# akanazawa/human_dynamics

Hardware: NVIDIA H100
Metric: frames/sec (ResNet->f_movie->SMPL LBS) (higher is better)
Workload: dtype f32 (wgmma 3x fp16 head/remainder split, fp32 two-level accumulate)

## Files before the change

human_dynamics_b200/_lib.py:

```python
from __future__ import annotations

import ctypes as C
import os

_HERE = os.path.dirname(os.path.abspath(__file__))
LIB_PATH = os.path.join(_HERE, 'libhd_b200.so')

HD_IMPL_SIMT, HD_IMPL_TC_3XTF32, HD_IMPL_TC_1XTF32, HD_IMPL_TC_3XF16 = 0, 1, 2, 3
HD_CONV_NO_TMA_EPILOGUE = 1
HD_CONV_INPUT_PLANES = 2
HD_PACK_FORWARD, HD_PACK_BACKWARD_DATA = 0, 1
IMPL_BY_NAME = {'simt': HD_IMPL_SIMT, 'tc3': HD_IMPL_TC_3XTF32, 'tc1': HD_IMPL_TC_1XTF32, 'tc3h': HD_IMPL_TC_3XF16}


class ConvDesc(C.Structure):
    _fields_ = [
        ('in_', C.c_void_p), ('in_ld', C.c_longlong),
        ('n_img', C.c_int), ('H', C.c_int), ('W', C.c_int), ('Cin', C.c_int),
        ('Ho', C.c_int), ('Wo', C.c_int), ('KH', C.c_int), ('KW', C.c_int),
        ('stride', C.c_int), ('pad_t', C.c_int), ('pad_l', C.c_int),
        ('w_kn', C.c_void_p), ('w_nk_hi', C.c_void_p), ('w_nk_lo', C.c_void_p),
        ('Cout', C.c_int), ('K_pad', C.c_int),
        ('pre_scale', C.c_void_p), ('pre_shift', C.c_void_p), ('pre_img_stride', C.c_int), ('pre_relu', C.c_int),
        ('post_scale', C.c_void_p), ('post_shift', C.c_void_p), ('post_relu', C.c_int),
        ('res', C.c_void_p), ('res_ld', C.c_longlong), ('res_H', C.c_int), ('res_W', C.c_int), ('res_stride', C.c_int),
        ('out', C.c_void_p), ('out_ld', C.c_longlong),
        ('impl', C.c_int),
        ('tmap_hi', C.c_void_p), ('tmap_lo', C.c_void_p),
        ('in_hi', C.c_void_p), ('in_lo', C.c_void_p),
        ('out_hi', C.c_void_p), ('out_lo', C.c_void_p), ('out2_ld', C.c_longlong),
        ('post2_scale', C.c_void_p), ('post2_shift', C.c_void_p), ('post2_relu', C.c_int),
        ('tmap_res', C.c_void_p), ('tmap_out', C.c_void_p), ('tmap_out_hi', C.c_void_p), ('tmap_out_lo', C.c_void_p),
        ('flags', C.c_int),
# ... 206 lines not shown
```

human_dynamics_b200/csrc/conv_common.cuh:

```cuda
#pragma once
#include <cuda_fp16.h>
#include "common.cuh"

namespace hd {

struct ConvParams {
  const float *in; long long in_ld;
  int n_img, H, W, Cin, Ho, Wo, KH, KW, stride, pad_t, pad_l;
  const float *w_kn; int Cout; int K; int M;
  const float *pre_scale, *pre_shift; int pre_img_stride, pre_relu;
  const float *post_scale, *post_shift; int post_relu;
  const float *res; long long res_ld; int res_H, res_W, res_stride;
  float *out; long long out_ld;
  int vec_out;
  int K_pad;
  const void *in_hi, *in_lo;
  void *out_hi, *out_lo; long long out2_ld;
  const float *post2_scale, *post2_shift; int post2_relu;
  int out_sub;
  int planes;
  long long *dbg;
};

#ifdef __CUDACC__
// ... 29 lines not shown
    return HD_ERR_INVALID;
  }
  p.in = d->in; p.in_ld = d->in_ld;
  p.n_img = d->n_img; p.H = d->H; p.W = d->W; p.Cin = d->Cin; p.Ho = d->Ho; p.Wo = d->Wo;
  p.KH = d->KH; p.KW = d->KW; p.stride = d->stride; p.pad_t = d->pad_t; p.pad_l = d->pad_l;
  p.w_kn = d->w_kn; p.Cout = d->Cout; p.K = d->KH * d->KW * d->Cin;
  const long long M = (long long)d->n_img * d->Ho * d->Wo;
  if (M > 0x7fffffffLL) { set_last_error_text("hd_conv_gemm: M overflows int32"); return HD_ERR_INVALID; }
  p.M = (int)M;
  p.pre_scale = d->pre_scale; p.pre_shift = d->pre_shift; p.pre_img_stride = d->pre_img_stride; p.pre_relu = d->pre_relu;
  p.post_scale = d->post_scale; p.post_shift = d->post_shift; p.post_relu = d->post_relu;
  p.res = d->res; p.res_ld = d->res_ld; p.res_H = d->res_H; p.res_W = d->res_W; p.res_stride = d->res_stride;
  p.out = d->out; p.out_ld = d->out_ld;
  p.in_hi = d->in_hi; p.in_lo = d->in_lo; p.out_hi = d->out_hi; p.out_lo = d->out_lo; p.out2_ld = d->out2_ld;
  p.post2_scale = d->post2_scale; p.post2_shift = d->post2_shift; p.post2_relu = d->post2_relu;
  p.vec_out = (d->Cout % 4 == 0) && (!d->out || ((d->out_ld % 4 == 0) && aligned16(d->out))) &&
              (!d->out_hi || ((d->out2_ld % 4 == 0) && aligned16(d->out_hi) && aligned16(d->out_lo))) &&
              (!d->res || ((d->res_ld % 4 == 0) && aligned16(d->res))) &&
              (!d->post_scale || aligned16(d->post_scale)) && (!d->post_shift || aligned16(d->post_shift));
  p.K_pad = d->K_pad;
  p.planes = (d->flags & HD_CONV_INPUT_PLANES) ? 1 : 0;
  p.out_sub = d->out_subsample > 1 ? d->out_subsample : 0;
  if (p.out_sub && !d->out) { set_last_error_text("hd_conv_gemm: out_subsample needs `out`"); return HD_ERR_INVALID; }
  p.dbg = nullptr;
  return HD_OK;
}

int launch_conv_simt(const ConvParams &p, cudaStream_t st);
int launch_conv_tc(const ConvParams &p, const hd_conv_desc *d, cudaStream_t st);

}
```

human_dynamics_b200/csrc/conv_tc.cu:

```cuda
#include <cuda.h>
#include <cuda_fp16.h>
#include <cstdlib>
#include "conv_common.cuh"
#include "tc_ptx.cuh"

namespace hd {
namespace {

constexpr int BM = 128;
constexpr int A_TILE_BYTES = BM * 128;
constexpr int BOX_BYTES = 64 * 128;
constexpr int W_PROD = 8;
constexpr int STAGE_OUT = 1, STAGE_PAIR = 2;

using namespace ptx;

template <bool HALF, bool ASPLIT, int BN, bool RES = false>
struct Cfg {
  static_assert(BN == 64 || (BN == 128 && HALF && ASPLIT), "128-wide N tiles: pre-split fp16 path only");
  static_assert(!RES || ASPLIT, "residual by TMA: pre-split fp16 path only");
  static constexpr int PROD_THREADS = BN == 128 ? 128 : 256;
  static constexpr int NUM_THREADS = 256 + PROD_THREADS;
  static constexpr int ROW_STEP = PROD_THREADS / 8;
  static constexpr int ROWS = BM / ROW_STEP;
  static constexpr int PROD_REGS = BN == 128 ? 40 : 104, CONS_REGS = BN == 128 ? 232 : 152;
  static_assert(256 * CONS_REGS + PROD_THREADS * PROD_REGS <= 65536, "setmaxnreg split beyond the register file");
  static constexpr int NACC = BN / 2;
  static constexpr int STAGES = BN == 128 ? (RES ? 2 : 3) : (RES ? 3 : 4);
  static constexpr int BKE = HALF ? 64 : 32;
  static constexpr int B_TILE_BYTES = BN * 128;
  static constexpr int STAGE_BYTES = 2 * A_TILE_BYTES + 2 * B_TILE_BYTES;
  static constexpr int RES_OFFSET = STAGES * STAGE_BYTES;
  static constexpr int RES_SLOT_BYTES = RES ? 64 * BN * 4 : 0;
  static constexpr int STG_OFFSET = RES_OFFSET + 2 * RES_SLOT_BYTES;
  static constexpr int STG_BYTES = ASPLIT ? 2 * BOX_BYTES : 0;
  static constexpr int BAR_OFFSET = STG_OFFSET + 2 * STG_BYTES;
  static constexpr int SMEM_BYTES = BAR_OFFSET + 128 + 1024;
  static_assert(SMEM_BYTES <= 232448, "dynamic shared memory beyond the 227 KB a CTA can opt into");
  static constexpr int PF = HALF ? 2 : 3;
  static constexpr int V = HALF ? 2 : 1;
};

template <int R>
struct RowState {
  int n[R], iy[R], ix[R];
};

template <bool SPLIT, int PCH, bool HALF, bool GATHER, bool ASPLIT, int BN, bool RES>
__global__ void __launch_bounds__((Cfg<HALF, ASPLIT, BN, RES>::NUM_THREADS), 1)
conv_gemm_tc_kernel(const ConvParams p, const __grid_constant__ CUtensorMap tmap_hi, const __grid_constant__ CUtensorMap tmap_lo,
                    const __grid_constant__ CUtensorMap tmap_res, const __grid_constant__ CUtensorMap tmap_out,
                    const __grid_constant__ CUtensorMap tmap_out_hi, const __grid_constant__ CUtensorMap tmap_out_lo, const int stage) {
  using C = Cfg<HALF, ASPLIT, BN, RES>;
  constexpr int BKE = C::BKE, PF = C::PF, V = C::V, STAGES = C::STAGES, R = C::ROWS, RS = C::ROW_STEP, NA = C::NACC;
  extern __shared__ uint8_t smem_raw[];
  const uint32_t smem_base = (smem_u32(smem_raw) + 1023u) & ~1023u;
  uint8_t *smem = smem_raw + (smem_base - smem_u32(smem_raw));
  const uint32_t bar_base = smem_base + C::BAR_OFFSET;
  auto full_bar = [&](int s) { return bar_base + 8u * s; };
  auto empty_bar = [&](int s) { return bar_base + 8u * (STAGES + s); };
  auto res_bar = [&](int g) { return bar_base + 8u * (2 * STAGES + g); };

  const int warp = threadIdx.x >> 5, lane = threadIdx.x & 31;
  const int num_k = (GATHER ? p.K_pad : p.K) / BKE;
  const int tiles_n = (p.Cout + BN - 1) / BN;
  const int num_tiles = ((p.M + BM - 1) / BM) * tiles_n;
  const int my_tiles = (num_tiles - (int)blockIdx.x + (int)gridDim.x - 1) / (int)gridDim.x;

  if (threadIdx.x == 0) {
    for (int s = 0; s < STAGES; ++s) {
      mbar_init(full_bar(s), ASPLIT ? C::PROD_THREADS + 1 : 9);
      mbar_init(empty_bar(s), 8);
    }
    if (RES) for (int g = 0; g < 2; ++g) mbar_init(res_bar(g), 1);
    asm volatile("fence.mbarrier_init.release.cluster;" ::: "memory");
  }
  __syncthreads();
  const int xmode = p.dbg ? (int)p.dbg[15] : 0;

  if (warp >= W_PROD) {
    asm volatile("setmaxnreg.dec.sync.aligned.u32 %0;" ::"n"(C::PROD_REGS));
    const int t = threadIdx.x - W_PROD * 32;
    const int j = t & 7;
    const int rb = t >> 3;
    const uint32_t sw_off = (uint32_t)((j ^ (rb & 7)) << 4);
    const bool prof = p.dbg != nullptr && blockIdx.x == 0 && t == 0;
    long long t_wait = 0, t_start = prof && BN == 64 ? clock64() : 0;
    if (BN == 128 && prof) p.dbg[0] = clock64();
    const int total = my_tiles * num_k;
    auto load_b = [&](int s, int ti, int kc) {
      if (t != 0) return;
      const int n0 = (((int)blockIdx.x + ti * (int)gridDim.x) % tiles_n) * BN;
      const uint32_t b_hi = smem_base + s * C::STAGE_BYTES + 2 * A_TILE_BYTES;
      if (xmode & 2) { mbar_arrive(full_bar(s)); return; }
      const int boxes = (BN == 128 && n0 + 64 < p.Cout) ? 2 : 1;
      mbar_arrive_expect_tx(full_bar(s), (SPLIT ? 2 : 1) * boxes * BOX_BYTES);
      for (int b = 0; b < boxes; ++b) {
// ... 2 lines not shown
      }
    };

    auto enter_tile = [&](int ti, RowState<R> &rs) {
      const int tile = (int)blockIdx.x + ti * (int)gridDim.x;
      const int m0 = (tile / tiles_n) * BM;
      const int hw = p.Ho * p.Wo;
#pragma unroll
      for (int i = 0; i < R; ++i) {
        const int m = m0 + rb + RS * i;
        if (m < p.M) {
          const int n = m / hw;
          const int r = m - n * hw;
          const int oy = r / p.Wo, ox = r - oy * p.Wo;
          rs.n[i] = n; rs.iy[i] = oy * p.stride - p.pad_t; rs.ix[i] = ox * p.stride - p.pad_l;
        } else {
          rs.n[i] = -1; rs.iy[i] = 0; rs.ix[i] = 0;
        }
      }
    };
    if constexpr (ASPLIT) {
      const __half *ihi = reinterpret_cast<const __half *>(p.in_hi);
      const __half *ilo = reinterpret_cast<const __half *>(p.in_lo);
      if (!p.planes && p.KH * p.KW <= 32 && (long long)p.n_img * p.H * p.W * p.in_ld < (1ll << 31)) {
        const uint32_t off0 = (uint32_t)rb * 128u + sw_off;
        int base[R];
        uint32_t mask[R];
        int kc = 0, ti = 0, tap = 0, ci0 = 0, kx = 0, ky = 0, tap_off = 0;
        for (int q = 0; q < total; ++q) {
          if (kc == 0) {
            const int tile = (int)blockIdx.x + ti * (int)gridDim.x;
            const int m0 = (tile / tiles_n) * BM + rb;
            const int hw = p.Ho * p.Wo;
#pragma unroll
            for (int i = 0; i < R; ++i) {
              const int m = m0 + RS * i;
              uint32_t mk = 0;
              int b = 0;
              if (m < p.M) {
                const int n = m / hw;
                const int r = m - n * hw;
                const int oy = r / p.Wo, ox = r - oy * p.Wo;
                const int iy0 = oy * p.stride - p.pad_t, ix0 = ox * p.stride - p.pad_l;
                b = ((n * p.H + iy0) * p.W + ix0) * p.in_ld + j * 8;
                int t = 0;
                for (int yy = 0; yy < p.KH; ++yy)
                  for (int xx = 0; xx < p.KW; ++xx, ++t)
// ... 577 lines not shown
}

constexpr int kMaxDevices = 64;

int encode_epilogue_map(CUtensorMap *tm, bool fp16, const void *base, int cols, int rows, long long ld_bytes, const char *what) {
  EncodeTiledFn fn = get_encode_fn();
  if (!fn) { set_last_error_text("cuTensorMapEncodeTiled unavailable (no CUDA driver?)"); return HD_ERR_UNSUPPORTED; }
  const cuuint64_t gdim[2] = {(cuuint64_t)cols, (cuuint64_t)rows};
  const cuuint64_t gstride[1] = {(cuuint64_t)ld_bytes};
  const cuuint32_t box[2] = {fp16 ? 64u : 32u, 64u};
  const cuuint32_t estr[2] = {1u, 1u};
  CUresult r = fn(tm, fp16 ? CU_TENSOR_MAP_DATA_TYPE_FLOAT16 : CU_TENSOR_MAP_DATA_TYPE_FLOAT32, 2, const_cast<void *>(base), gdim, gstride,
                  box, estr, CU_TENSOR_MAP_INTERLEAVE_NONE, CU_TENSOR_MAP_SWIZZLE_128B, CU_TENSOR_MAP_L2_PROMOTION_L2_128B,
                  CU_TENSOR_MAP_FLOAT_OOB_FILL_NONE);
  if (r != CUDA_SUCCESS) {
    char msg[96];
    snprintf(msg, sizeof(msg), "cuTensorMapEncodeTiled (%s) failed with CUresult %d", what, (int)r);
    set_last_error_text(msg);
    return HD_ERR_CUDA;
  }
  return HD_OK;
}

template <bool SPLIT, int PCH, bool HALF, bool GATHER = false, bool ASPLIT = false, int BN = 64, bool RES = false>
int launch_tc(const ConvParams &p, const hd_conv_desc *d, cudaStream_t st) {
  using C = Cfg<HALF, ASPLIT, BN, RES>;
  static bool configured[kMaxDevices] = {};
  static int num_sms[kMaxDevices] = {};
  int dev = 0;
  cudaGetDevice(&dev);
  if (dev < 0 || dev >= kMaxDevices) { set_last_error_text("conv_gemm_tc: device ordinal out of range"); return HD_ERR_UNSUPPORTED; }
  if (!configured[dev]) {
    cudaError_t e = cudaFuncSetAttribute(conv_gemm_tc_kernel<SPLIT, PCH, HALF, GATHER, ASPLIT, BN, RES>,
                                         cudaFuncAttributeMaxDynamicSharedMemorySize, C::SMEM_BYTES);
    if (e != cudaSuccess) { set_last_error("conv_gemm_tc attr", e); return HD_ERR_CUDA; }
    cudaDeviceGetAttribute(&num_sms[dev], cudaDevAttrMultiProcessorCount, dev);
    if (num_sms[dev] <= 0) { set_last_error_text("conv_gemm_tc: no multiprocessor count"); return HD_ERR_CUDA; }
    configured[dev] = true;
  }
  alignas(64) CUtensorMap thi, tlo;
  const void *mhi = d->tmap_hi_n64 ? d->tmap_hi_n64 : d->tmap_hi;
  const void *mlo = d->tmap_hi_n64 ? d->tmap_lo_n64 : d->tmap_lo;
  memcpy(&thi, mhi, sizeof(CUtensorMap));
  memcpy(&tlo, mlo ? mlo : mhi, sizeof(CUtensorMap));
  alignas(64) CUtensorMap tres, tout, tohi, tolo;
  memcpy(&tres, &thi, sizeof(CUtensorMap));
  memcpy(&tout, &thi, sizeof(CUtensorMap));
  memcpy(&tohi, &thi, sizeof(CUtensorMap));
  memcpy(&tolo, &thi, sizeof(CUtensorMap));
  int rc = HD_OK;
  if (RES) rc = encode_epilogue_map(&tres, false, p.res, p.Cout, p.M, p.res_ld * 4, "residual");
  int stage = 0;
  if (ASPLIT && p.out && !p.out_sub) {
    stage |= STAGE_OUT;
    if (rc == HD_OK) rc = encode_epilogue_map(&tout, false, p.out, p.Cout, p.M, p.out_ld * 4, "output");
  }
  if (ASPLIT && p.out_hi && p.out2_ld % 8 == 0) {
    stage |= STAGE_PAIR;
    if (rc == HD_OK) rc = encode_epilogue_map(&tohi, true, p.out_hi, p.Cout, p.M, p.out2_ld * 2, "output head");
    if (rc == HD_OK) rc = encode_epilogue_map(&tolo, true, p.out_lo, p.Cout, p.M, p.out2_ld * 2, "output remainder");
  }
  if (rc != HD_OK) return rc;
  const int num_tiles = ceil_div(p.M, BM) * ceil_div(p.Cout, BN);
  dim3 grid(num_tiles < num_sms[dev] ? num_tiles : num_sms[dev]);
  conv_gemm_tc_kernel<SPLIT, PCH, HALF, GATHER, ASPLIT, BN, RES>
      <<<grid, C::NUM_THREADS, C::SMEM_BYTES, st>>>(p, thi, tlo, tres, tout, tohi, tolo, stage);
  return check_launch("conv_gemm_tc_kernel");
}

bool wide_n_tile(const ConvParams &p) {
  if (p.Cout <= 64) return false;
  int dev = 0, sms = 0;
  cudaGetDevice(&dev);
  cudaDeviceGetAttribute(&sms, cudaDevAttrMultiProcessorCount, dev);
  if (sms <= 0) return true;
  const long long m_tiles = ceil_div(p.M, BM);
  const long long w128 = (m_tiles * ceil_div(p.Cout, 128) + sms - 1) / sms, w64 = (m_tiles * ceil_div(p.Cout, 64) + sms - 1) / sms;
  return 16 * w128 <= 9 * w64;
}

}

int launch_conv_tc(const ConvParams &p, const hd_conv_desc *d, cudaStream_t st) {
  const bool split_b = d->impl != HD_IMPL_TC_1XTF32;
  if (!d->tmap_hi || (split_b && !d->tmap_lo) || (!d->tmap_hi_n64 && d->tmap_lo_n64) || (d->tmap_hi_n64 && split_b && !d->tmap_lo_n64)) {
    set_last_error_text("hd_conv_gemm(tc): missing tensor maps (tmap_hi/tmap_lo, and tmap_hi_n64/tmap_lo_n64 together or not at all)");
    return HD_ERR_INVALID;
  }
  const bool half = d->impl == HD_IMPL_TC_3XF16;
  const int bke = half ? 64 : 32;
  if (p.out_sub) {
    const bool res_plain = !p.res || (p.res_stride == 1 && p.res_H == p.Ho && p.res_W == p.Wo);
    const bool maps = (!p.res || d->tmap_res) && (!p.out_hi || (d->tmap_out_hi && d->tmap_out_lo));
    if (!p.in_hi || p.planes || !maps || !res_plain || p.Cout % 32 != 0 || (d->flags & HD_CONV_NO_TMA_EPILOGUE)) {
      set_last_error_text("hd_conv_gemm: out_subsample needs the activation-map epilogue (pre-split input, Cout % 32 == 0, activation maps given)");
      return HD_ERR_UNSUPPORTED;
    }
  }
  if ((p.out_hi || p.in_hi) && (!half || !p.vec_out)) {
    set_last_error_text("hd_conv_gemm(tc): pre-split activations need impl 3 and 16-byte aligned, 4-column-multiple outputs");
    return HD_ERR_INVALID;
  }
  if (p.in_hi && p.planes) {
    if (p.Cin != 32 || p.KH != 8 || p.KW != 1 || p.stride != 2 || p.pad_t != 0 || p.pad_l != 0 || p.in_ld != 4 || p.Cout > 64 ||
        p.W % 2 != 0 || 2 * (p.Wo - 1) + 8 > p.W || 2 * (p.Ho - 1) + 7 > p.H || !aligned16(p.in_hi) || !aligned16(p.in_lo) || p.pre_scale) {
      set_last_error_text("hd_conv_gemm(tc planes): needs the conv1 plane geometry (Cin 32, KH 8, KW 1, stride 2, in_ld 4, even W)");
      return HD_ERR_INVALID;
    }
    return launch_tc<true, 2, true, false, true>(p, d, st);
  }
  if (p.in_hi) {
    if (p.Cin % 64 != 0 || p.K % 64 != 0 || p.in_ld % 8 != 0 || !aligned16(p.in_hi) || !aligned16(p.in_lo) || p.pre_scale) {
      set_last_error_text("hd_conv_gemm(tc split-A): needs Cin % 64 == 0, in_ld % 8 == 0, aligned in_hi/in_lo, no prologue");
      return HD_ERR_INVALID;
    }
    const bool res_rows = p.res && p.res_stride == 1 && p.res_H == p.Ho && p.res_W == p.Wo && p.K <= 8 * 64;
    if (wide_n_tile(p))
      return res_rows ? launch_tc<true, 2, true, false, true, 128, true>(p, d, st) : launch_tc<true, 2, true, false, true, 128>(p, d, st);
    return res_rows ? launch_tc<true, 2, true, false, true, 64, true>(p, d, st) : launch_tc<true, 2, true, false, true>(p, d, st);
  }
  if (half && p.Cin % bke != 0) {
    const int segp = (p.KW * p.Cin + 7) & ~7;
    if (p.K_pad % 64 != 0 || p.K_pad < p.KH * segp || p.Cout > 64 || p.pre_scale || p.in_ld != p.Cin) {
      set_last_error_text("hd_conv_gemm(tc gather): needs K_pad % 64 == 0, K_pad >= KH*roundup8(KW*Cin), Cout <= 64, dense pixels, no prologue");
      return HD_ERR_INVALID;
    }
    return launch_tc<true, 2, true, true>(p, d, st);
  }
  if (!p.in || p.Cin % bke != 0 || p.in_ld % 4 != 0 || !aligned16(p.in) || p.K % bke != 0 ||
      (p.pre_scale && (!aligned16(p.pre_scale) || !aligned16(p.pre_shift) || p.pre_img_stride % 4 != 0))) {
    set_last_error_text("hd_conv_gemm(tc): needs Cin % 32 (tf32) / % 64 (fp16) == 0 and 16-byte aligned input / prologue vectors");
    return HD_ERR_INVALID;
// ... 55 lines not shown
```

human_dynamics_b200/csrc/net_plan.cu:

```cuda
#include "common.cuh"

#include <algorithm>
#include <cmath>
#include <cstdint>
#include <deque>
#include <functional>
#include <string>
#include <utility>
#include <vector>

struct hd_net {
  int kind = 0;
  hd_weight_fn get = nullptr;
  void *user = nullptr;
  std::vector<void *> allocs;
  std::deque<std::vector<unsigned char>> wmaps;
  std::deque<std::vector<unsigned char>> maps;
  std::vector<std::function<int(cudaStream_t)>> steps;
  std::string err;
  const float *in0 = nullptr;
  float *out0 = nullptr, *out1 = nullptr;
  int n = 0, size = 0, B = 0, T = 0, C = 0, layers = 0, N = 0, D = 0;
  const float *bound_in = nullptr;
  float *bound_out = nullptr;
// ... 101 lines not shown
    c.stride = stride; c.pad_t = pad_t; c.pad_l = pad_l; c.post_relu = relu;
    if (!w) w = weight(wname, (long long)c.K * Cout);
    if (!w) return false;
    std::vector<float> w_kn(w, w + (size_t)c.K * Cout);
    c.w_kn = (float *)upload(w_kn);
    if (scale) c.post_scale = (float *)upload(*scale);
    if (shift) c.post_shift = (float *)upload(*shift);
    if (!c.w_kn || (scale && !c.post_scale) || (shift && !c.post_shift)) return false;
    if (!tc) return true;
    if (Cin % 64 != 0) return fail(HD_ERR_UNSUPPORTED, "layer '" + wname + "': Cin % 64 != 0 has no fp16 tensor-core packing");
    return pack(c, c.w_kn, KH * KW, Cin);
  }

  bool bias_vec(const std::string &name, int C, std::vector<float> &v) {
    const float *b = weight(name, C);
    if (!b) return false;
    v.assign(b, b + C);
    return true;
  }

  struct Bind {
    int n = 0, H = 0, W = 0;
    Pair in;
    float *out = nullptr;
    Pair out2;
    const float *post2_scale = nullptr, *post2_shift = nullptr;
    int post2_relu = 0;
    const float *res = nullptr;
    long long res_ld = 0;
    int res_H = 0, res_W = 0, res_stride = 1;
    int out_subsample = 0;
  };

  bool bind(const PackedConv &c, const Bind &b, hd_conv_desc &d) {
    memset(&d, 0, sizeof(d));
    const int Ho = c.KH > 1 ? (b.H + 2 * c.pad_t - c.KH) / c.stride + 1 : (b.H - 1) / c.stride + 1;
    const int Wo = c.KW > 1 ? (b.W + 2 * c.pad_l - c.KW) / c.stride + 1 : (b.W - 1) / c.stride + 1;
    d.in_ld = c.Cin;
    d.in_hi = b.in.hi; d.in_lo = b.in.lo;
    d.n_img = b.n; d.H = b.H; d.W = b.W; d.Cin = c.Cin; d.Ho = Ho; d.Wo = Wo; d.KH = c.KH; d.KW = c.KW;
    d.stride = c.stride; d.pad_t = c.pad_t; d.pad_l = c.pad_l;
    d.w_kn = c.w_kn; d.Cout = c.Cout; d.K_pad = c.K_pad;
    d.post_scale = c.post_scale; d.post_shift = c.post_shift; d.post_relu = c.post_relu;
    if (b.res) { d.res = b.res; d.res_ld = b.res_ld; d.res_H = b.res_H; d.res_W = b.res_W; d.res_stride = b.res_stride; }
    d.out = b.out; d.out_ld = c.Cout;
    d.out_subsample = b.out ? b.out_subsample : 0;
    if (b.out2.hi) {
      d.out_hi = b.out2.hi; d.out_lo = b.out2.lo; d.out2_ld = c.Cout;
      d.post2_scale = b.post2_scale; d.post2_shift = b.post2_shift; d.post2_relu = b.post2_relu;
    }
    d.impl = HD_IMPL_TC_3XF16;
    d.w_nk_hi = c.w_hi; d.w_nk_lo = c.w_lo; d.tmap_hi = c.tmap_hi; d.tmap_lo = c.tmap_lo;
    return encode_act_maps(d);
  }

  bool encode_act_maps(hd_conv_desc &d) {
    d.tmap_res = d.tmap_out = d.tmap_out_hi = d.tmap_out_lo = nullptr;
    const bool ok = d.impl == HD_IMPL_TC_3XF16 && d.in_hi && d.Cout % 32 == 0 &&
                    (!d.res || (d.res_stride == 1 && d.res_H == d.Ho && d.res_W == d.Wo));
    if (!ok) return true;
    const long long M = (long long)d.n_img * d.Ho * d.Wo;
    struct F { const void *ptr; long long ld; int eb; const void **slot; };
// ... 165 lines not shown
  if (b.rc != HD_OK) { const int r = b.rc; hd_net_destroy(net); return r; }

  net->steps.push_back([=](cudaStream_t st) { return hd_pack_conv1_planes(net->in0, plane_hi, plane_lo, n, size, size, WP, (void *)st); });
  {
    hd_conv_desc d;
    memset(&d, 0, sizeof(d));
    d.in_hi = plane_hi; d.in_lo = plane_lo; d.in_ld = 4;
    d.n_img = n; d.H = size + 6; d.W = WP; d.Cin = 32; d.Ho = d.Wo = H1;
    d.KH = 8; d.KW = 1; d.stride = 2; d.pad_t = 0; d.pad_l = 0; d.Cout = 64; d.K_pad = 256;
    d.post_shift = conv1.post_shift; d.out = bufS; d.out_ld = 64; d.impl = HD_IMPL_TC_3XF16;
    d.w_nk_hi = conv1.w_hi; d.w_nk_lo = conv1.w_lo; d.tmap_hi = conv1.tmap_hi; d.tmap_lo = conv1.tmap_lo;
    d.flags = HD_CONV_INPUT_PLANES;
    if (!b.encode_act_maps(d)) { const int r = b.rc; hd_net_destroy(net); return r; }
    b.conv_step(d);
  }
  {
    const float *ps = units[0].pre_scale, *pb = units[0].pre_shift;
    float *pool_out = units[0].has_shortcut ? nullptr : bufA;
    net->steps.push_back([=](cudaStream_t st) { return hd_maxpool3x3s2_same(bufS, pool_out, n, H1, H1, 64, ps, pb, xs.hi, xs.lo, (void *)st); });
  }
  float *x = bufA, *y = bufB;
  int H = H2;
  bool sub_ready = false;
  for (size_t ui = 0; ui < units.size() && b.rc == HD_OK; ++ui) {
    const Unit &un = units[ui];
    const int s = un.stride, Ho = (H - 1) / s + 1;
    const float *res = nullptr;
    hd_conv_desc d;
    if (un.has_shortcut) {
      Builder::Bind bs; bs.n = n; bs.H = H; bs.W = H; bs.in = xs; bs.out = bufS;
      if (!b.bind(un.shortcut, bs, d)) break;
      b.conv_step(d);
      res = bufS;
    } else if (s > 1) {
      if (!sub_ready) {
        const float *src = x;
        const int Hh = H, Cc = un.depth;
        net->steps.push_back([=](cudaStream_t st) { return hd_subsample(src, bufS, n, Hh, Hh, Cc, s, (void *)st); });
      }
      res = bufS;
    } else {
      res = x;
    }
    Builder::Bind b1; b1.n = n; b1.H = H; b1.W = H; b1.in = xs; b1.out2 = r1;
    if (!b.bind(un.conv1, b1, d)) break;
    b.conv_step(d);
    Builder::Bind b2; b2.n = n; b2.H = H; b2.W = H; b2.in = r1; b2.out2 = r2;
    if (!b.bind(un.conv2, b2, d)) break;
    b.conv_step(d);
    const bool last = ui + 1 == units.size();
    Builder::Bind b3; b3.n = n; b3.H = Ho; b3.W = Ho; b3.in = r2;
    b3.res = res; b3.res_ld = un.depth; b3.res_H = Ho; b3.res_W = Ho; b3.res_stride = 1;
    sub_ready = false;
    if (!last) {
      b3.out2 = ys; b3.post2_scale = units[ui + 1].pre_scale; b3.post2_shift = units[ui + 1].pre_shift; b3.post2_relu = 1;
      b3.out = units[ui + 1].has_shortcut ? nullptr : y;
      if (b3.out && units[ui + 1].stride > 1 && !un.has_shortcut && s == 1) {
        sub_ready = true;
        b3.out = bufS; b3.out_subsample = units[ui + 1].stride;
      }
    } else {
      b3.out = y;
    }
    if (!b.bind(un.conv3, b3, d)) break;
    b.conv_step(d);
    std::swap(x, y);
    std::swap(xs, ys);
    H = Ho;
  }
  if (b.rc != HD_OK) { const int r = b.rc; hd_net_destroy(net); return r; }
  {
    const float *fin = x;
    const int HW = H * H, Cc = d_in;
    net->steps.push_back([=](cudaStream_t st) { return hd_bnrelu_avgpool(fin, post_scale, post_shift, net->out0, n, HW, Cc, (void *)st); });
  }
  *out_net = net;
  return HD_OK;
// ... 124 lines not shown
```

human_dynamics_b200/nets.py:

```python
from __future__ import annotations

import ctypes as C
import os

import numpy as np
import torch

from . import _lib
from ._lib import lib, check, fptr, current_stream, ConvDesc

RESNET_BLOCKS = ((64, 3, 2), (128, 4, 2), (256, 6, 2), (512, 3, 1))
BN_EPS = 1e-5
GN_EPS = 1e-6
GN_GROUPS = 32


def _dev(a, device, dtype=np.float32):
    if isinstance(a, torch.Tensor):
        return a
    return torch.from_numpy(np.ascontiguousarray(a, dtype=dtype)).to(device)


def pack_weight(src, KH, Cin, Cout, hi, lo, stream):
    check(lib.hd_pack_weight(C.c_void_p(src.data_ptr()), KH, Cin, Cout, _lib.HD_PACK_FORWARD, hi.element_size(), C.c_void_p(hi.data_ptr()),
# ... 52 lines not shown
            seg = self.KW * self.Cin
            segp = (seg + 7) // 8 * 8
            self.K_pad = (self.KH * segp + 63) // 64 * 64 if gather else self.K
            if gather:
                src = torch.zeros((self.KH, segp, self.Cout), dtype=torch.float32, device=device)
                src[:, :seg] = self.w_kn.view(self.KH, seg, self.Cout)
                self.pack_src = (src, self.KH, segp)
            else:
                self.pack_src = (self.w_kn, self.KH * self.KW, self.Cin)
            rows = (self.Cout + 63) // 64 * 64
            dt = torch.float16 if want == 'f16' else torch.float32
            self.w_nk_hi = torch.empty((rows, self.K_pad), dtype=dt, device=device)
            self.w_nk_lo = torch.empty((rows, self.K_pad), dtype=dt, device=device)
            if _packs_on(device):
                self.repack(current_stream())
            self.tmap_hi, self.tmap_lo = weight_tmap(self.w_nk_hi), weight_tmap(self.w_nk_lo)
            self.tc = want

    def repack(self, stream):
        src, KH, Cin = self.pack_src
        pack_weight(src, KH, Cin, self.Cout, self.w_nk_hi, self.w_nk_lo, stream)

    def bind(self, inp, n_img, H, W, out, in_ld=None, out_ld=None, pre=None, res=None, res_geom=None, impl='auto',
             inp_split=None, out_split=None, post2=None, out_subsample=0):
        d = ConvDesc()
        Ho = (H + 2 * self.pad_t - self.KH) // self.stride + 1 if self.KH > 1 else (H - 1) // self.stride + 1
        Wo = (W + 2 * self.pad_l - self.KW) // self.stride + 1 if self.KW > 1 else (W - 1) // self.stride + 1
        d.in_ = inp.data_ptr() if inp is not None else None
        d.in_ld = self.Cin if in_ld is None else in_ld
        if inp_split is not None:
            d.in_hi, d.in_lo = inp_split[0].data_ptr(), inp_split[1].data_ptr()
        d.n_img, d.H, d.W, d.Cin = n_img, H, W, self.Cin
        d.Ho, d.Wo, d.KH, d.KW = Ho, Wo, self.KH, self.KW
        d.stride, d.pad_t, d.pad_l = self.stride, self.pad_t, self.pad_l
        d.w_kn = self.w_kn.data_ptr()
        d.Cout = self.Cout
        d.K_pad = self.K_pad
        if pre is not None:
            d.pre_scale, d.pre_shift = pre[0].data_ptr(), pre[1].data_ptr()
            d.pre_img_stride, d.pre_relu = int(pre[2]), int(pre[3])
        if self.post_scale is not None:
            d.post_scale = self.post_scale.data_ptr()
        if self.post_shift is not None:
            d.post_shift = self.post_shift.data_ptr()
        d.post_relu = int(self.post_relu)
        if res is not None:
            d.res = res.data_ptr()
# ... 6 lines not shown
        if out_split is not None:
            d.out_hi, d.out_lo, d.out2_ld = out_split[0].data_ptr(), out_split[1].data_ptr(), self.Cout
            if post2 is not None:
                if post2[0] is not None:
                    d.post2_scale = post2[0].data_ptr()
                if post2[1] is not None:
                    d.post2_shift = post2[1].data_ptr()
                d.post2_relu = int(post2[2])
        use_tc = bool(self.tc) and impl in ('auto', 'tc3', 'tc1', 'tc3h') and \
            (self.gather or inp_split is not None or ((d.in_ld % 4 == 0) and (inp.data_ptr() % 16 == 0)))
        if (inp_split is not None or out_split is not None) and not (use_tc and self.tc == 'f16'):
            raise _lib.HDError('pre-split activations need the fp16 tensor-core packing (impl auto / tc3h, Cin % 64 == 0)')
        if use_tc:
            if self.tc == 'f16':
                d.impl = _lib.HD_IMPL_TC_3XF16
            else:
                d.impl = _lib.HD_IMPL_TC_1XTF32 if impl == 'tc1' else _lib.HD_IMPL_TC_3XTF32
            d.w_nk_hi, d.w_nk_lo = self.w_nk_hi.data_ptr(), self.w_nk_lo.data_ptr()
            d.tmap_hi = C.cast(self.tmap_hi, C.c_void_p)
            d.tmap_lo = C.cast(self.tmap_lo, C.c_void_p)
        else:
            d.impl = _lib.HD_IMPL_SIMT
        op = ConvOp(d, (self, inp, out, pre, res, inp_split, out_split, post2), (Ho, Wo))
        if not TMA_EPILOGUE:
            d.flags |= _lib.HD_CONV_NO_TMA_EPILOGUE
        op.encode_act_maps()
        return op


class SubsampleOp(object):
    __slots__ = ('src', 'dst', 'geom', 'd')

    def __init__(self, src, dst, n, H, C, stride):
        self.src, self.dst, self.geom, self.d = src, dst, (n, H, H, C, stride), None

    def rebind(self, field, tensor):
        self.src = tensor

    def encode_act_maps(self):
        pass

    def run(self, stream):
        n, H, W, Cc, s = self.geom
        check(lib.hd_subsample(fptr(self.src), fptr(self.dst), n, H, W, Cc, s, stream), 'hd_subsample')


# ... 27 lines not shown
                               ('out_lo', d.out_lo, d.out2_ld, 2)):
            if not ptr or (f == 'out' and d.out_subsample > 1):
                continue
            if ptr % 16 or (ld * eb) % 16:
                for g in ('tmap_res', 'tmap_out', 'tmap_out_hi', 'tmap_out_lo'):
                    setattr(d, g, None)
                return
            check(lib.hd_make_act_tmap(C.c_void_p(ptr), M, d.Cout, ld, eb, C.cast(self.maps[f], C.c_void_p)), 'hd_make_act_tmap')
            setattr(d, 'tmap_' + f, C.cast(self.maps[f], C.c_void_p))

    def rebind(self, field, tensor):
        setattr(self.d, field, tensor.data_ptr())
        self.dyn[field] = tensor

    def run(self, stream):
        rc = lib.hd_conv_gemm(self.ref, stream)
        if rc:
            check(rc, 'hd_conv_gemm')


DROP_DEAD_FP32 = os.environ.get('HD_DROP_DEAD_FP32', '1') != '0'
FAST_HEADS = os.environ.get('HD_FAST_HEADS', '1') != '0'
CONV1_PLANES = os.environ.get('HD_CONV1_PLANES', '1') != '0'


class PackedConv1Planes(object):

    def __init__(self, w_hwio, bias, device):
        w = np.asarray(w_hwio, np.float32)
        assert w.shape == (7, 7, 3, 64), w.shape
        self.device = device
        self.Cout, self.K = 64, 256
        wp = np.zeros((8, 8, 4, 64), np.float32)
        wp[:7, :7, :3] = w
        self.w_nk_hi = torch.empty((64, 256), dtype=torch.float16, device=device)
        self.w_nk_lo = torch.empty((64, 256), dtype=torch.float16, device=device)
        if _packs_on(device):
            pack_weight(_dev(wp, device), 8, 32, 64, self.w_nk_hi, self.w_nk_lo, current_stream())
        self.bias = _dev(bias, device)
        self.tmap_hi, self.tmap_lo = weight_tmap(self.w_nk_hi), weight_tmap(self.w_nk_lo)

    @staticmethod
    def plane_width(size):
        return (size + 8 + 1) // 2 * 2

    def alloc_planes(self, n, size):
# ... 94 lines not shown
        self.conv1_op = None
        self.planes = None
        if root and packed.conv1_planes is not None and impl in ('auto', 'tc3h') and CONV1_PLANES and size % 2 == 0:
            self.planes = packed.conv1_planes.alloc_planes(n, size)
            self.conv1_op = packed.conv1_planes.bind(self.planes, n, size, self.bufS)
        elif root and packed.conv1.tc and impl != 'simt':
            self.conv1_op = packed.conv1.bind(self.bufS, n, size, size, self.bufS, in_ld=3, impl=impl)
        self.in_refs = []
        self.pool_split = None
        self.pool_f32_dead = False
        x, y = self.bufA, self.bufB
        units = packed.units[lo:hi]
        if self.split:
            def pair(count):
                return (torch.empty(max(1, count), **f16), torch.empty(max(1, count), **f16))
            xs, ys = pair(n * mx_io), pair(n * mx_io)
            r1, r2 = pair(n * mx_r), pair(n * mx_r)
            self.in_split = xs
            if root:
                self.pool_split = (units[0]['pre'][0], units[0]['pre'][1], xs)
                self.pool_f32_dead = DROP_DEAD_FP32 and 'shortcut' in units[0]
            self.out_split = None
            sub_ready = False
            for ui, unit in enumerate(units):
                s = unit['stride']
                Ho = (H - 1) // s + 1
                if 'shortcut' in unit:
                    self.ops.append(unit['shortcut'].bind(None, n, H, H, self.bufS, inp_split=xs, impl=impl))
                    if ui == 0:
                        self.in_refs += [(self.ops[-1], 'in_hi', 0), (self.ops[-1], 'in_lo', 1)]
                    res, res_geom = self.bufS, (unit['depth'], Ho, Ho, 1)
                elif s > 1 and SUBSAMPLE_RES:
                    if not sub_ready:
                        self.ops.append(SubsampleOp(x, self.bufS[:n * Ho * Ho * unit['depth']], n, H, unit['depth'], s))
                        if ui == 0:
                            self.in_refs.append((self.ops[-1], 'res', 2))
                    res, res_geom = self.bufS, (unit['depth'], Ho, Ho, 1)
                else:
                    res, res_geom = x, (unit['depth'], H, H, s)
                self.ops.append(unit['conv1'].bind(None, n, H, H, None, inp_split=xs, out_split=r1, impl=impl))
                if ui == 0:
                    self.in_refs += [(self.ops[-1], 'in_hi', 0), (self.ops[-1], 'in_lo', 1)]
                self.ops.append(unit['conv2'].bind(None, n, H, H, None, inp_split=r1, out_split=r2, impl=impl))
                last = ui == len(units) - 1
                nxt = units[ui + 1]['pre'] if not last else next_pre
                osplit = ys if nxt is not None else None
                nxt_conv_shortcut = ('shortcut' in units[ui + 1]) if not last else bool(next_has_shortcut)
                y_out = None if (osplit is not None and nxt_conv_shortcut and DROP_DEAD_FP32) else y
                s_next = units[ui + 1]['stride'] if not last else 1
                sub_ready = bool(SUBSAMPLE_EPI and SUBSAMPLE_RES and not last and s_next > 1 and 'shortcut' not in units[ui + 1] and
                                 'shortcut' not in unit and s == 1 and y_out is not None and osplit is not None)
                if sub_ready:
                    y_out = self.bufS
                self.ops.append(unit['conv3'].bind(None, n, Ho, Ho, y_out, inp_split=r2, res=res, res_geom=res_geom, impl=impl,
                                                   out_split=osplit, post2=(nxt[0], nxt[1], 1) if nxt is not None else None,
                                                   out_subsample=s_next if sub_ready else 0))
                if ui == 0 and 'shortcut' not in unit and not (s > 1 and SUBSAMPLE_RES):
                    self.in_refs.append((self.ops[-1], 'res', 2))
                if last:
                    self.out_split = osplit
                x, y = y, x
                xs, ys = ys, xs
                H = Ho
                d_in = unit['depth']
        else:
            self.bufR1 = torch.empty(max(1, n * mx_r), **f32)
            self.bufR2 = torch.empty(max(1, n * mx_r), **f32)
            for ui, unit in enumerate(units):
# ... 306 lines not shown
```

include/hd_b200.h:

```cpp
#ifndef HD_B200_H_
#define HD_B200_H_

#include <stddef.h>
#include <stdint.h>

#ifdef __cplusplus
extern "C" {
#endif

typedef enum {
  HD_OK = 0,
  HD_ERR_INVALID = 1,
  HD_ERR_WORKSPACE = 2,
  HD_ERR_CUDA = 3,
  HD_ERR_UNSUPPORTED = 4
} hd_status;

int hd_version(void);
const char *hd_status_string(int status);
const char *hd_last_error(void);
long long hd_launch_count(void);
void hd_launch_count_reset(void);

enum { HD_IMPL_SIMT = 0, HD_IMPL_TC_3XTF32 = 1, HD_IMPL_TC_1XTF32 = 2, HD_IMPL_TC_3XF16 = 3 };
// ... 3 lines not shown
  int n_img, H, W, Cin;
  int Ho, Wo, KH, KW, stride, pad_t, pad_l;
  const float *w_kn;
  const void *w_nk_hi;
  const void *w_nk_lo;
  int Cout;  int K_pad;
  const float *pre_scale, *pre_shift;  int pre_img_stride;  int pre_relu;
  const float *post_scale, *post_shift;  int post_relu;
  const float *res;  long long res_ld;  int res_H, res_W, res_stride;
  float *out;  long long out_ld;
  int impl;
  const void *tmap_hi, *tmap_lo;
  const void *in_hi, *in_lo;
  void *out_hi, *out_lo;  long long out2_ld;
  const float *post2_scale, *post2_shift;  int post2_relu;
  const void *tmap_res, *tmap_out, *tmap_out_hi, *tmap_out_lo;
  int flags;
  const void *tmap_hi_n64, *tmap_lo_n64;
  int out_subsample;
} hd_conv_desc;

enum {
  HD_CONV_NO_TMA_EPILOGUE = 1,
  HD_CONV_INPUT_PLANES = 2
};

int hd_conv_gemm(const hd_conv_desc *d, void *stream);
int hd_conv_gemm_profile(const hd_conv_desc *d, void *stream, long long *dbg);

int hd_make_weight_tmap(const void *w_nk, int rows, int k_pad, int box_rows, int elem_bytes, void *tmap_out);
int hd_make_act_tmap(const void *base, long long rows, int cols, long long ld_elems, int elem_bytes, void *tmap_out);

int hd_pack_conv1_planes(const float *img, void *plane_hi, void *plane_lo, int N, int H, int W, int WP, void *stream);
int hd_conv1_7x7s2(const float *in, const float *w, const float *bias, float *out, int N, int H, int W, void *stream);
int hd_maxpool3x3s2_same(const float *in, float *out, int N, int H, int W, int C, const float *scale, const float *shift,
                         void *out_hi, void *out_lo, void *stream);
int hd_subsample(const float *in, float *out, int N, int H, int W, int C, int stride, void *stream);
int hd_bnrelu_avgpool(const float *in, const float *scale, const float *shift, float *out, int N, int HW, int C, void *stream);

int hd_process_image(const unsigned char *frames, int N, int H, int W, const int *geom, float *out, int S, void *plane_hi,
                     void *plane_lo, int WP, void *stream);
int hd_crop_geometry(int H, int W, const double *bbox, int img_size, int *geom, int *center, int *start_pt);

#define HD_AUG_SRC_U8 1
#define HD_AUG_ROTATE 2
#define HD_AUG_FLIP 4
typedef struct {
// ... 196 lines not shown
```

Before: 12910.

## Feed fp32 activations into 1x1 conv via TMA and split to fp16 in-kernel

For large identity-shortcut bottleneck units, the previous conv3 no longer writes a pre-activated fp16 hi/lo pair. The next conv1 instead TMA-loads the raw fp32 output into extra shared-memory slots. Its producer warps then apply BN scale/shift and ReLU and split the values into fp16 hi/lo tiles. This drops the write and re-read of the doubled split tensor for big activations, at the cost of fewer pipeline stages, more shared memory and extra producer work per k-step.

```diff
diff --git a/human_dynamics_b200/_lib.py b/human_dynamics_b200/_lib.py
--- a/human_dynamics_b200/_lib.py
+++ b/human_dynamics_b200/_lib.py
@@ -9,6 +9,7 @@
 HD_IMPL_SIMT, HD_IMPL_TC_3XTF32, HD_IMPL_TC_1XTF32, HD_IMPL_TC_3XF16 = 0, 1, 2, 3
 HD_CONV_NO_TMA_EPILOGUE = 1
 HD_CONV_INPUT_PLANES = 2
+HD_CONV_INPUT_F32_PREACT = 4
 HD_PACK_FORWARD, HD_PACK_BACKWARD_DATA = 0, 1
 IMPL_BY_NAME = {'simt': HD_IMPL_SIMT, 'tc3': HD_IMPL_TC_3XTF32, 'tc1': HD_IMPL_TC_1XTF32, 'tc3h': HD_IMPL_TC_3XF16}
 
diff --git a/human_dynamics_b200/csrc/conv_common.cuh b/human_dynamics_b200/csrc/conv_common.cuh
--- a/human_dynamics_b200/csrc/conv_common.cuh
+++ b/human_dynamics_b200/csrc/conv_common.cuh
@@ -75,6 +75,18 @@
   p.planes = (d->flags & HD_CONV_INPUT_PLANES) ? 1 : 0;
   p.out_sub = d->out_subsample > 1 ? d->out_subsample : 0;
   if (p.out_sub && !d->out) { set_last_error_text("hd_conv_gemm: out_subsample needs `out`"); return HD_ERR_INVALID; }
+  if (d->flags & HD_CONV_INPUT_F32_PREACT) {
+    const bool ok = d->in && !d->in_hi && !d->in_lo && d->pre_scale && d->pre_img_stride == 0 && aligned16(d->pre_scale) &&
+                    aligned16(d->pre_shift) && d->KH == 1 && d->KW == 1 && d->stride == 1 && d->pad_t == 0 && d->pad_l == 0 &&
+                    d->H == d->Ho && d->W == d->Wo && d->impl == HD_IMPL_TC_3XF16 && d->Cin % 64 == 0 && d->in_ld % 4 == 0 &&
+                    aligned16(d->in) && !(d->flags & HD_CONV_INPUT_PLANES) && p.vec_out;
+    if (!ok) {
+      set_last_error_text("hd_conv_gemm: HD_CONV_INPUT_F32_PREACT needs impl 3, a 1x1 stride-1 unpadded conv, fp32 `in` (no in_hi/in_lo) "
+                          "with a 16-byte aligned base and row pitch, Cin % 64 == 0, per-channel pre_scale/pre_shift (pre_img_stride 0) "
+                          "and 16-byte aligned, 4-column-multiple outputs");
+      return HD_ERR_INVALID;
+    }
+  }
   p.dbg = nullptr;
   return HD_OK;
 }
diff --git a/human_dynamics_b200/csrc/conv_tc.cu b/human_dynamics_b200/csrc/conv_tc.cu
--- a/human_dynamics_b200/csrc/conv_tc.cu
+++ b/human_dynamics_b200/csrc/conv_tc.cu
@@ -15,10 +15,11 @@
 
 using namespace ptx;
 
-template <bool HALF, bool ASPLIT, int BN, bool RES = false>
+template <bool HALF, bool ASPLIT, int BN, bool RES = false, bool F32A = false>
 struct Cfg {
   static_assert(BN == 64 || (BN == 128 && HALF && ASPLIT), "128-wide N tiles: pre-split fp16 path only");
   static_assert(!RES || ASPLIT, "residual by TMA: pre-split fp16 path only");
+  static_assert(!F32A || (ASPLIT && !RES), "fp32 pre-activated input: the pre-split layout and epilogue, no TMA residual");
   static constexpr int PROD_THREADS = BN == 128 ? 128 : 256;
   static constexpr int NUM_THREADS = 256 + PROD_THREADS;
   static constexpr int ROW_STEP = PROD_THREADS / 8;
@@ -26,11 +27,14 @@
   static constexpr int PROD_REGS = BN == 128 ? 40 : 104, CONS_REGS = BN == 128 ? 232 : 152;
   static_assert(256 * CONS_REGS + PROD_THREADS * PROD_REGS <= 65536, "setmaxnreg split beyond the register file");
   static constexpr int NACC = BN / 2;
-  static constexpr int STAGES = BN == 128 ? (RES ? 2 : 3) : (RES ? 3 : 4);
+  static constexpr int STAGES = F32A ? 2 : BN == 128 ? (RES ? 2 : 3) : (RES ? 3 : 4);
   static constexpr int BKE = HALF ? 64 : 32;
   static constexpr int B_TILE_BYTES = BN * 128;
   static constexpr int STAGE_BYTES = 2 * A_TILE_BYTES + 2 * B_TILE_BYTES;
-  static constexpr int RES_OFFSET = STAGES * STAGE_BYTES;
+  static constexpr int RAW_SLOTS = F32A ? (BN == 128 ? 2 : 3) : 0;
+  static constexpr int RAW_SLOT_BYTES = 4 * BOX_BYTES;
+  static constexpr int RAW_OFFSET = STAGES * STAGE_BYTES;
+  static constexpr int RES_OFFSET = RAW_OFFSET + RAW_SLOTS * RAW_SLOT_BYTES;
   static constexpr int RES_SLOT_BYTES = RES ? 64 * BN * 4 : 0;
   static constexpr int STG_OFFSET = RES_OFFSET + 2 * RES_SLOT_BYTES;
   static constexpr int STG_BYTES = ASPLIT ? 2 * BOX_BYTES : 0;
@@ -46,12 +50,13 @@
   int n[R], iy[R], ix[R];
 };
 
-template <bool SPLIT, int PCH, bool HALF, bool GATHER, bool ASPLIT, int BN, bool RES>
-__global__ void __launch_bounds__((Cfg<HALF, ASPLIT, BN, RES>::NUM_THREADS), 1)
+template <bool SPLIT, int PCH, bool HALF, bool GATHER, bool ASPLIT, int BN, bool RES, bool F32A>
+__global__ void __launch_bounds__((Cfg<HALF, ASPLIT, BN, RES, F32A>::NUM_THREADS), 1)
 conv_gemm_tc_kernel(const ConvParams p, const __grid_constant__ CUtensorMap tmap_hi, const __grid_constant__ CUtensorMap tmap_lo,
                     const __grid_constant__ CUtensorMap tmap_res, const __grid_constant__ CUtensorMap tmap_out,
-                    const __grid_constant__ CUtensorMap tmap_out_hi, const __grid_constant__ CUtensorMap tmap_out_lo, const int stage) {
-  using C = Cfg<HALF, ASPLIT, BN, RES>;
+                    const __grid_constant__ CUtensorMap tmap_out_hi, const __grid_constant__ CUtensorMap tmap_out_lo,
+                    const __grid_constant__ CUtensorMap tmap_in, const int stage) {
+  using C = Cfg<HALF, ASPLIT, BN, RES, F32A>;
   constexpr int BKE = C::BKE, PF = C::PF, V = C::V, STAGES = C::STAGES, R = C::ROWS, RS = C::ROW_STEP, NA = C::NACC;
   extern __shared__ uint8_t smem_raw[];
   const uint32_t smem_base = (smem_u32(smem_raw) + 1023u) & ~1023u;
@@ -60,6 +65,7 @@
   auto full_bar = [&](int s) { return bar_base + 8u * s; };
   auto empty_bar = [&](int s) { return bar_base + 8u * (STAGES + s); };
   auto res_bar = [&](int g) { return bar_base + 8u * (2 * STAGES + g); };
+  auto raw_bar = [&](int r) { return bar_base + 8u * (2 * STAGES + 2 + r); };
 
   const int warp = threadIdx.x >> 5, lane = threadIdx.x & 31;
   const int num_k = (GATHER ? p.K_pad : p.K) / BKE;
@@ -73,6 +79,7 @@
       mbar_init(empty_bar(s), 8);
     }
     if (RES) for (int g = 0; g < 2; ++g) mbar_init(res_bar(g), 1);
+    for (int r = 0; r < C::RAW_SLOTS; ++r) mbar_init(raw_bar(r), 1);
     asm volatile("fence.mbarrier_init.release.cluster;" ::: "memory");
   }
   __syncthreads();
@@ -121,7 +128,58 @@
     if constexpr (ASPLIT) {
       const __half *ihi = reinterpret_cast<const __half *>(p.in_hi);
       const __half *ilo = reinterpret_cast<const __half *>(p.in_lo);
-      if (!p.planes && p.KH * p.KW <= 32 && (long long)p.n_img * p.H * p.W * p.in_ld < (1ll << 31)) {
+      if constexpr (F32A) {
+        constexpr int NR = C::RAW_SLOTS;
+        const uint32_t raw0 = smem_base + C::RAW_OFFSET;
+        auto load_raw = [&](int q) {
+          if (t != 0 || q >= total) return;
+          const int ti = q / num_k, kc = q - ti * num_k;
+          const int m0 = (((int)blockIdx.x + ti * (int)gridDim.x) / tiles_n) * BM;
+          const int halves = m0 + 64 < p.M ? 2 : 1;
+          const uint32_t dst = raw0 + (q % NR) * C::RAW_SLOT_BYTES;
+          mbar_arrive_expect_tx(raw_bar(q % NR), 2 * halves * BOX_BYTES);
+          for (int h = 0; h < 2; ++h)
+            for (int rh = 0; rh < halves; ++rh)
+              tma_load_2d(dst + h * 2 * BOX_BYTES + rh * BOX_BYTES, &tmap_in, raw_bar(q % NR), kc * BKE + 32 * h, m0 + 64 * rh);
+        };
+        constexpr int RS2 = C::PROD_THREADS / 16, R2 = BM / RS2;
+        const int hp = t & 15, rr = t >> 4;
+        const uint32_t rsw = (uint32_t)(rr & 7);
+        const uint8_t *raw_t = smem + C::RAW_OFFSET + (hp >> 3) * 2 * BOX_BYTES + rr * 128 + ((((uint32_t)hp & 7u) ^ rsw) << 4);
+        const uint32_t st_off = (uint32_t)rr * 128u + ((((uint32_t)hp >> 1) ^ rsw) << 4) + 8u * (hp & 1);
+        for (int u = 0; u < NR; ++u) load_raw(u);
+        int kc = 0, ti = 0;
+        for (int q = 0; q < total; ++q) {
+          const int s = q % STAGES;
+          const uint32_t ph = (uint32_t)(q / STAGES) & 1u;
+          long long tw0 = prof ? clock64() : 0;
+          mbar_wait(empty_bar(s), ph ^ 1u);
+          if (prof) t_wait += clock64() - tw0;
+          load_b(s, ti, kc);
+          const float4 sc = __ldg(reinterpret_cast<const float4 *>(p.pre_scale + kc * BKE + 4 * hp));
+          const float4 sh = __ldg(reinterpret_cast<const float4 *>(p.pre_shift + kc * BKE + 4 * hp));
+          mbar_wait(raw_bar(q % NR), (uint32_t)(q / NR) & 1u);
+          const uint8_t *src = raw_t + (q % NR) * C::RAW_SLOT_BYTES;
+          uint8_t *dst = smem + s * C::STAGE_BYTES + st_off;
+#pragma unroll
+          for (int i = 0; i < R2; ++i) {
+            const float4 x = *reinterpret_cast<const float4 *>(src + i * RS2 * 128);
+            float a0 = __fadd_rn(__fmul_rn(x.x, sc.x), sh.x), a1 = __fadd_rn(__fmul_rn(x.y, sc.y), sh.y);
+            float a2 = __fadd_rn(__fmul_rn(x.z, sc.z), sh.z), a3 = __fadd_rn(__fmul_rn(x.w, sc.w), sh.w);
+            if (p.pre_relu) { a0 = fmaxf(a0, 0.f); a1 = fmaxf(a1, 0.f); a2 = fmaxf(a2, 0.f); a3 = fmaxf(a3, 0.f); }
+            uint32_t h0, h1, l0, l1;
+            split_f16x2(a0, a1, h0, l0);
+            split_f16x2(a2, a3, h1, l1);
+            *reinterpret_cast<uint2 *>(dst + i * RS2 * 128) = make_uint2(h0, h1);
+            *reinterpret_cast<uint2 *>(dst + A_TILE_BYTES + i * RS2 * 128) = make_uint2(l0, l1);
+          }
+          fence_proxy_async();
+          mbar_arrive(full_bar(s));
+          named_bar_sync(5, C::PROD_THREADS);
+          load_raw(q + NR);
+          if (++kc == num_k) { kc = 0; ++ti; }
+        }
+      } else if (!p.planes && p.KH * p.KW <= 32 && (long long)p.n_img * p.H * p.W * p.in_ld < (1ll << 31)) {
         const uint32_t off0 = (uint32_t)rb * 128u + sw_off;
         int base[R];
         uint32_t mask[R];
@@ -745,16 +803,16 @@
   return HD_OK;
 }
 
-template <bool SPLIT, int PCH, bool HALF, bool GATHER = false, bool ASPLIT = false, int BN = 64, bool RES = false>
+template <bool SPLIT, int PCH, bool HALF, bool GATHER = false, bool ASPLIT = false, int BN = 64, bool RES = false, bool F32A = false>
 int launch_tc(const ConvParams &p, const hd_conv_desc *d, cudaStream_t st) {
-  using C = Cfg<HALF, ASPLIT, BN, RES>;
+  using C = Cfg<HALF, ASPLIT, BN, RES, F32A>;
   static bool configured[kMaxDevices] = {};
   static int num_sms[kMaxDevices] = {};
   int dev = 0;
   cudaGetDevice(&dev);
   if (dev < 0 || dev >= kMaxDevices) { set_last_error_text("conv_gemm_tc: device ordinal out of range"); return HD_ERR_UNSUPPORTED; }
   if (!configured[dev]) {
-    cudaError_t e = cudaFuncSetAttribute(conv_gemm_tc_kernel<SPLIT, PCH, HALF, GATHER, ASPLIT, BN, RES>,
+    cudaError_t e = cudaFuncSetAttribute(conv_gemm_tc_kernel<SPLIT, PCH, HALF, GATHER, ASPLIT, BN, RES, F32A>,
                                          cudaFuncAttributeMaxDynamicSharedMemorySize, C::SMEM_BYTES);
     if (e != cudaSuccess) { set_last_error("conv_gemm_tc attr", e); return HD_ERR_CUDA; }
     cudaDeviceGetAttribute(&num_sms[dev], cudaDevAttrMultiProcessorCount, dev);
@@ -766,13 +824,15 @@
   const void *mlo = d->tmap_hi_n64 ? d->tmap_lo_n64 : d->tmap_lo;
   memcpy(&thi, mhi, sizeof(CUtensorMap));
   memcpy(&tlo, mlo ? mlo : mhi, sizeof(CUtensorMap));
-  alignas(64) CUtensorMap tres, tout, tohi, tolo;
+  alignas(64) CUtensorMap tres, tout, tohi, tolo, tin;
   memcpy(&tres, &thi, sizeof(CUtensorMap));
   memcpy(&tout, &thi, sizeof(CUtensorMap));
   memcpy(&tohi, &thi, sizeof(CUtensorMap));
   memcpy(&tolo, &thi, sizeof(CUtensorMap));
+  memcpy(&tin, &thi, sizeof(CUtensorMap));
   int rc = HD_OK;
   if (RES) rc = encode_epilogue_map(&tres, false, p.res, p.Cout, p.M, p.res_ld * 4, "residual");
+  if (F32A && rc == HD_OK) rc = encode_epilogue_map(&tin, false, p.in, p.Cin, p.M, p.in_ld * 4, "input");
   int stage = 0;
   if (ASPLIT && p.out && !p.out_sub) {
     stage |= STAGE_OUT;
@@ -786,8 +846,8 @@
   if (rc != HD_OK) return rc;
   const int num_tiles = ceil_div(p.M, BM) * ceil_div(p.Cout, BN);
   dim3 grid(num_tiles < num_sms[dev] ? num_tiles : num_sms[dev]);
-  conv_gemm_tc_kernel<SPLIT, PCH, HALF, GATHER, ASPLIT, BN, RES>
-      <<<grid, C::NUM_THREADS, C::SMEM_BYTES, st>>>(p, thi, tlo, tres, tout, tohi, tolo, stage);
+  conv_gemm_tc_kernel<SPLIT, PCH, HALF, GATHER, ASPLIT, BN, RES, F32A>
+      <<<grid, C::NUM_THREADS, C::SMEM_BYTES, st>>>(p, thi, tlo, tres, tout, tohi, tolo, tin, stage);
   return check_launch("conv_gemm_tc_kernel");
 }
 
@@ -831,6 +891,10 @@
       return HD_ERR_INVALID;
     }
     return launch_tc<true, 2, true, false, true>(p, d, st);
+  }
+  if (d->flags & HD_CONV_INPUT_F32_PREACT) {
+    if (wide_n_tile(p)) return launch_tc<true, 2, true, false, true, 128, false, true>(p, d, st);
+    return launch_tc<true, 2, true, false, true, 64, false, true>(p, d, st);
   }
   if (p.in_hi) {
     if (p.Cin % 64 != 0 || p.K % 64 != 0 || p.in_ld % 8 != 0 || !aligned16(p.in_hi) || !aligned16(p.in_lo) || p.pre_scale) {
diff --git a/human_dynamics_b200/csrc/net_plan.cu b/human_dynamics_b200/csrc/net_plan.cu
--- a/human_dynamics_b200/csrc/net_plan.cu
+++ b/human_dynamics_b200/csrc/net_plan.cu
@@ -147,6 +147,7 @@
   struct Bind {
     int n = 0, H = 0, W = 0;
     Pair in;
+    const float *in_f32 = nullptr, *pre_scale = nullptr, *pre_shift = nullptr;
     float *out = nullptr;
     Pair out2;
     const float *post2_scale = nullptr, *post2_shift = nullptr;
@@ -162,7 +163,11 @@
     const int Ho = c.KH > 1 ? (b.H + 2 * c.pad_t - c.KH) / c.stride + 1 : (b.H - 1) / c.stride + 1;
     const int Wo = c.KW > 1 ? (b.W + 2 * c.pad_l - c.KW) / c.stride + 1 : (b.W - 1) / c.stride + 1;
     d.in_ld = c.Cin;
-    d.in_hi = b.in.hi; d.in_lo = b.in.lo;
+    if (b.in_f32) {
+      d.in = b.in_f32; d.pre_scale = b.pre_scale; d.pre_shift = b.pre_shift; d.pre_relu = 1; d.flags = HD_CONV_INPUT_F32_PREACT;
+    } else {
+      d.in_hi = b.in.hi; d.in_lo = b.in.lo;
+    }
     d.n_img = b.n; d.H = b.H; d.W = b.W; d.Cin = c.Cin; d.Ho = Ho; d.Wo = Wo; d.KH = c.KH; d.KW = c.KW;
     d.stride = c.stride; d.pad_t = c.pad_t; d.pad_l = c.pad_l;
     d.w_kn = c.w_kn; d.Cout = c.Cout; d.K_pad = c.K_pad;
@@ -374,6 +379,7 @@
   float *x = bufA, *y = bufB;
   int H = H2;
   bool sub_ready = false;
+  bool in_f32 = false;
   for (size_t ui = 0; ui < units.size() && b.rc == HD_OK; ++ui) {
     const Unit &un = units[ui];
     const int s = un.stride, Ho = (H - 1) / s + 1;
@@ -395,6 +401,7 @@
       res = x;
     }
     Builder::Bind b1; b1.n = n; b1.H = H; b1.W = H; b1.in = xs; b1.out2 = r1;
+    if (in_f32) { b1.in_f32 = x; b1.pre_scale = un.pre_scale; b1.pre_shift = un.pre_shift; }
     if (!b.bind(un.conv1, b1, d)) break;
     b.conv_step(d);
     Builder::Bind b2; b2.n = n; b2.H = H; b2.W = H; b2.in = r1; b2.out2 = r2;
@@ -404,7 +411,10 @@
     Builder::Bind b3; b3.n = n; b3.H = Ho; b3.W = Ho; b3.in = r2;
     b3.res = res; b3.res_ld = un.depth; b3.res_H = Ho; b3.res_W = Ho; b3.res_stride = 1;
     sub_ready = false;
-    if (!last) {
+    in_f32 = !last && !units[ui + 1].has_shortcut && units[ui + 1].stride == 1 && 4ll * n * Ho * Ho * un.depth > (50ll << 20);
+    if (in_f32) {
+      b3.out = y;
+    } else if (!last) {
       b3.out2 = ys; b3.post2_scale = units[ui + 1].pre_scale; b3.post2_shift = units[ui + 1].pre_shift; b3.post2_relu = 1;
       b3.out = units[ui + 1].has_shortcut ? nullptr : y;
       if (b3.out && units[ui + 1].stride > 1 && !un.has_shortcut && s == 1) {
diff --git a/human_dynamics_b200/nets.py b/human_dynamics_b200/nets.py
--- a/human_dynamics_b200/nets.py
+++ b/human_dynamics_b200/nets.py
@@ -98,7 +98,7 @@
         pack_weight(src, KH, Cin, self.Cout, self.w_nk_hi, self.w_nk_lo, stream)
 
     def bind(self, inp, n_img, H, W, out, in_ld=None, out_ld=None, pre=None, res=None, res_geom=None, impl='auto',
-             inp_split=None, out_split=None, post2=None, out_subsample=0):
+             inp_split=None, out_split=None, post2=None, out_subsample=0, flags=0):
         d = ConvDesc()
         Ho = (H + 2 * self.pad_t - self.KH) // self.stride + 1 if self.KH > 1 else (H - 1) // self.stride + 1
         Wo = (W + 2 * self.pad_l - self.KW) // self.stride + 1 if self.KW > 1 else (W - 1) // self.stride + 1
@@ -151,6 +151,7 @@
         else:
             d.impl = _lib.HD_IMPL_SIMT
         op = ConvOp(d, (self, inp, out, pre, res, inp_split, out_split, post2), (Ho, Wo))
+        d.flags |= flags
         if not TMA_EPILOGUE:
             d.flags |= _lib.HD_CONV_NO_TMA_EPILOGUE
         op.encode_act_maps()
@@ -224,6 +225,8 @@
 DROP_DEAD_FP32 = os.environ.get('HD_DROP_DEAD_FP32', '1') != '0'
 FAST_HEADS = os.environ.get('HD_FAST_HEADS', '1') != '0'
 CONV1_PLANES = os.environ.get('HD_CONV1_PLANES', '1') != '0'
+F32_PREACT = os.environ.get('HD_F32_PREACT', '1') != '0'
+F32_PREACT_MIN_PAIR_BYTES = 50 << 20
 
 
 class PackedConv1Planes(object):
@@ -364,6 +367,7 @@
                 self.pool_f32_dead = DROP_DEAD_FP32 and 'shortcut' in units[0]
             self.out_split = None
             sub_ready = False
+            in_f32 = False
             for ui, unit in enumerate(units):
                 s = unit['stride']
                 Ho = (H - 1) // s + 1
@@ -380,12 +384,20 @@
                     res, res_geom = self.bufS, (unit['depth'], Ho, Ho, 1)
                 else:
                     res, res_geom = x, (unit['depth'], H, H, s)
-                self.ops.append(unit['conv1'].bind(None, n, H, H, None, inp_split=xs, out_split=r1, impl=impl))
+                if in_f32:
+                    self.ops.append(unit['conv1'].bind(x, n, H, H, None, pre=(unit['pre'][0], unit['pre'][1], 0, 1), out_split=r1,
+                                                       impl=impl, flags=_lib.HD_CONV_INPUT_F32_PREACT))
+                else:
+                    self.ops.append(unit['conv1'].bind(None, n, H, H, None, inp_split=xs, out_split=r1, impl=impl))
                 if ui == 0:
                     self.in_refs += [(self.ops[-1], 'in_hi', 0), (self.ops[-1], 'in_lo', 1)]
                 self.ops.append(unit['conv2'].bind(None, n, H, H, None, inp_split=r1, out_split=r2, impl=impl))
                 last = ui == len(units) - 1
                 nxt = units[ui + 1]['pre'] if not last else next_pre
+                in_f32 = bool(F32_PREACT and not last and 'shortcut' not in units[ui + 1] and units[ui + 1]['stride'] == 1 and
+                              4 * n * Ho * Ho * unit['depth'] > F32_PREACT_MIN_PAIR_BYTES)
+                if in_f32:
+                    nxt = None
                 osplit = ys if nxt is not None else None
                 nxt_conv_shortcut = ('shortcut' in units[ui + 1]) if not last else bool(next_has_shortcut)
                 y_out = None if (osplit is not None and nxt_conv_shortcut and DROP_DEAD_FP32) else y
diff --git a/include/hd_b200.h b/include/hd_b200.h
--- a/include/hd_b200.h
+++ b/include/hd_b200.h
@@ -49,7 +49,8 @@
 
 enum {
   HD_CONV_NO_TMA_EPILOGUE = 1,
-  HD_CONV_INPUT_PLANES = 2
+  HD_CONV_INPUT_PLANES = 2,
+  HD_CONV_INPUT_F32_PREACT = 4
 };
 
 int hd_conv_gemm(const hd_conv_desc *d, void *stream);
```

Measured after the change: 13290 (median of 6 runs). +3.0%, better.
